# duylebkHCM/doc2tex

Measured on AMD Instinct MI355X. Metric: formulas/s (greedy decode, 128x512 crops), higher is better.
Workload: dtype bf16x3

## Files before the change

doc2tex_amd/_lib.py:

```python
import ctypes as C
import os

_HERE = os.path.dirname(os.path.abspath(__file__))
LIB_PATH = os.path.join(_HERE, "csrc", "libd2t.so")
if os.environ.get("D2T_PROBE_LIB"):
    LIB_PATH = os.path.abspath(os.environ["D2T_PROBE_LIB"])

D2T_OK = 0
D2T_EINVAL, D2T_ENOMEM, D2T_EHIP, D2T_ESTATE = 1, 2, 3, 4
ENC_RESNET, ENC_HYBRID_VIT, ENC_VGG_BILSTM, ENC_RESNET_BILSTM, ENC_VGG = 0, 1, 2, 3, 4
DEC_TFM, DEC_ATTN = 0, 1
ATTN_KEYS_ALL_INIT_MEAN, ATTN_KEYS_NOCLS_INIT_CLS, ATTN_KEYS_ALL_INIT_FIRST = 0, 1, 2
ACT_NONE, ACT_RELU, ACT_GELU = 0, 1, 2
CONV_FP32, CONV_BF16X3, CONV_FP16X2, CONV_MIXED = 0, 1, 2, 3
ATTN_CELL_LOCATION, ATTN_CELL_BAHDANAU = 0, 1
VIT_POS_SINCOS_PREFIX, VIT_POS_LEARNED_INTERP, VIT_POS_LEARNED_PREFIX = 0, 1, 2


class D2TConfig(C.Structure):
    _fields_ = [(n, C.c_int32) for n in (
        "encoder", "in_channels", "backbone_out", "vit_depth", "vit_heads", "vit_dim", "patch_h", "patch_w",
        "max_h", "max_w", "dec_dim", "dec_heads", "dec_layers", "dec_ff", "vocab", "max_seq_len",
        "decoder", "attn_hidden", "attn_kernel_size", "attn_kernel_dim", "attn_keys", "attn_enc_init",
        "attn_coverage", "bilstm_hidden", "batch_max_length", "gcb", "attn_cell", "attn_onehot", "vit_pos",
# ... 95 lines not shown
    "d2t_decode_beam": (_I, [_P, _P, _I, _I, C.POINTER(C.c_int64), C.POINTER(_I), C.POINTER(C.c_float), _P]),
    "d2t_decode_beam_batch": (_I, [_P, _P, _I, _I, _I, C.POINTER(C.c_int64), C.POINTER(_I), C.POINTER(C.c_float), _P]),
    "d2t_decode_beam_batch_ragged": (_I, [_P, _P, _I, C.POINTER(_I), _I, C.POINTER(C.c_int64), C.POINTER(_I), C.POINTER(C.c_float),
                                          _P]),
    "d2t_decode_supports_ragged_beam": (_I, [_P]),
    "d2t_ragged_beam_tables": (_L, [_I, C.POINTER(_I), C.POINTER(_I), C.POINTER(_I)]),
    "d2t_decode_attn_beam_batch": (_I, [_P, _P, _I, _I, _I, C.POINTER(C.c_int64), C.POINTER(_I), C.POINTER(C.c_float), _P]),
    "d2t_decode_attn_beam_batch_alpha": (_I, [_P, _P, _I, _I, _I, C.POINTER(C.c_int64), C.POINTER(_I), C.POINTER(C.c_float), _P,
                                               _P]),
    "d2t_decode_attn_beam_batch_ragged": (_I, [_P, _P, _I, C.POINTER(_I), _I, C.POINTER(C.c_int64), C.POINTER(_I),
                                               C.POINTER(C.c_float), _P, _P]),
    "d2t_decode_attn_supports_ragged_beam": (_I, [_P]),
    "d2t_decode_attn_beam": (_I, [_P, _P, _I, _I, C.POINTER(C.c_int64), C.POINTER(_I), C.POINTER(C.c_float), _P]),
    "d2t_decode_attn_supports_device_beam": (_I, [_P]),
    "d2t_set_attn_beam_device": (_I, [_P, _I]),
    "d2t_decode_attn_beam_device_runs": (_L, [_P]),
    "d2t_decode_attn_beam_batch_submit": (_I, [_P, _P, _I, C.POINTER(_I), _I, _P, _P, _P, _P, _P, C.POINTER(_L)]),
    "d2t_set_conv_precision": (_I, [_P, _I]),
    "d2t_set_mixed_units": (_I, [_P, _I]),
    "d2t_set_reserved_blocks": (_I, [_P, _I]),
    "d2t_set_decode_chains": (_I, [_P, _I]),
    "d2t_set_conv_kernel": (_I, [_P, _I]),
    "d2t_set_conv_fusion": (_I, [_P, _I, _I]),
    "d2t_set_beam_shared_tile": (_I, [_P, _I]),
    "d2t_set_reserved_cus": (_I, [_P, _I]),
    "d2t_train_forward": (_I, [_P, _P, _I, _I, _I, _P, _I, _P, _P]),
    "d2t_train_backward": (_I, [_P, _P, _P]),
    "d2t_train_grad": (_I, [_P, C.c_char_p, _P, C.c_int64, _P]),
    "d2t_reload_weights": (_I, [_P, _I, C.POINTER(C.c_char_p), C.POINTER(C.c_void_p), C.POINTER(C.c_int64), _P]),
    "d2t_train_gather": (_I, [_P, _I, _I, C.POINTER(C.c_char_p), C.POINTER(C.c_int64), C.POINTER(C.c_int64), _P, _P]),
    "d2t_read_weight": (_I, [_P, C.c_char_p, _P, C.c_int64, _P]),
    "d2t_train_set_dropout": (_I, [_P, C.c_float, C.c_uint64]),
    "d2t_train_set_teacher_flags": (_I, [_P, C.c_char_p, _I]),
    "d2t_train_mask_count": (_I, [_P]),
    "d2t_train_decision_count": (_I, [_P]),
    "d2t_train_read_decision": (_I, [_P, _I, _P, C.c_int64, C.POINTER(_I), C.POINTER(C.c_int64), _P]),
    "d2t_train_read_mask": (_I, [_P, _I, _P, C.c_int64, _P]),
    "d2t_train_read_attn_alpha": (_I, [_P, _P, C.c_int64, _P]),
    "d2t_train_release": (None, [_P]),
    "d2t_profile_enable": (_I, [_P, _I]),
    "d2t_profile_read": (_I, [_P, _I, C.POINTER(_I)] + [C.POINTER(_I)] * 3 + [C.POINTER(C.c_float)]),
    "d2t_op_conv2d": (_I, [_P] * 5 + [_I] * 12 + [_P]),
    "d2t_op_conv2d_bf16x3": (_I, [_P] * 5 + [_I] * 12 + [_P]),
    "d2t_op_conv2d_bf16x3_split": (_I, [_P] * 5 + [_I] * 12 + [_P]),
    "d2t_op_conv2d_bf16x3_split_pool": (_I, [_P] * 4 + [_I] * 12 + [_P]),
    "d2t_op_set_conv_kernel": (_I, [_I, _I]),
    "d2t_op_linear": (_I, [_P] * 5 + [_I] * 4 + [_P]),
    "d2t_op_maxpool2x2": (_I, [_P, _P] + [_I] * 8 + [_P]),
    "d2t_op_layernorm": (_I, [_P] * 4 + [_I, _I, C.c_float, _P]),
    "d2t_op_vit_attention": (_I, [_P, _P, _I, _I, _I, _P]),
    "d2t_op_vit_attention_probs": (_I, [_P, _P, _P, _I, _I, _I, _P]),
    "d2t_op_decode_attention": (_I, [_P] * 4 + [_I] * 5 + [_P]),
    "d2t_op_skinny": (_I, [_P] * 6 + [C.c_float, _P, _P] + [_I] * 6 + [_P, _L, _P]),
    "d2t_op_decoder_row": (_I, [_I] + [_P] * 13 + [C.c_float, _P, _P] + [_I] * 7 + [_P, _P, _I, _P, _I, _P]),
    "d2t_op_decoder_row_ragged": (_I, [_I] + [_P] * 13 + [C.c_float, _P, _P] + [_I] * 4 + [C.POINTER(_I), C.POINTER(_I), _P]),
    "d2t_op_decoder_row_ragged_beam": (_I, [_I] + [_P] * 13 + [C.c_float, _P, _P] + [_I] * 5 +
                                       [C.POINTER(_I), C.POINTER(_I), _P, _P, _I, _P]),
    "d2t_op_argmax_embed": (_I, [_P, _I] + [_P] * 13 + [_I] * 6 + [_P]),
    "d2t_op_beam_topk": (_I, [_P, _P, _P] + [_I] * 4 + [_P, _P, _P]),
    "d2t_op_beam_advance": (_I, [_I, _L] + [_P] * 15 + [_I] * 6 + [_P]),
    "d2t_op_beam_ancestry": (_I, [_P, _P, _P, _I, _I, _P, _P, _P, _P, _P]),
    "d2t_op_cache_gather": (_I, [_P, _P, _P] + [_I] * 7 + [_P]),
    "d2t_op_records_split": (_I, [_P, _P, _L, _I, _I, _P]),
    "d2t_op_records_merge": (_I, [_P, _P, _L, _I, _I, _P]),
    "d2t_op_conv_records": (_I, [C.POINTER(D2TOpConvRecordsArgs), _P]),
    "d2t_op_linear_kv": (_I, [_P] * 4 + [_I] * 7 + [_P]),
    "d2t_op_maxpool_records": (_I, [_P, _P] + [_I] * 9 + [_P]),
    "d2t_op_stem_records": (_I, [_P] * 4 + [_I] * 6 + [_P]),
    "d2t_op_pack_conv": (_I, [_P] * 6 + [C.c_float] + [_P] * 6 + [_I] * 4 + [_P]),
    "d2t_ce_forward": (_I, [_P, _P, _P, _P, _I, _I, _L, _P]),
    "d2t_ce_backward": (_I, [_P, _P, _P, _P, _P, _I, _I, _L, _P]),
    "d2t_ce_smooth_forward": (_I, [_P] * 6 + [_I, _I, _L, C.c_float, C.c_float, _I, _L, _P]),
    "d2t_ce_smooth_backward": (_I, [_P] * 7 + [_I, _I, _L, C.c_float, C.c_float, _I, _L, _P]),
    "d2t_optim_create": (_I, [C.POINTER(_P)]),
    "d2t_optim_destroy": (None, [_P]),
    "d2t_optim_last_error": (C.c_char_p, [_P]),
    "d2t_optim_chunk": (_I, []),
    "d2t_optim_step": (_I, [_P, C.POINTER(D2TOptimTensor), _I, _I, C.c_float, _P, _P]),
    "d2t_weight_ptr": (_I, [_P, C.c_char_p, C.POINTER(_P), C.POINTER(_L)]),
    "d2t_metric_edit_distance_workspace": (_I, [_I, _L, C.POINTER(_L)]),
    "d2t_metric_edit_distance": (_I, [_P, _P, _L, _P, _P, _L, _P, _I, _L, _P, _L, _P]),
    "d2t_metric_bleu_counts": (_I, [_P, _I, _P, _I, _I, _L, _I, _P, _P]),
    "d2t_op_train_conv": (_I, [_P] * 14 + [_I] * 13 + [_P]),
    "d2t_op_train_linear": (_I, [_P] * 10 + [_I] * 5 + [_P]),
    "d2t_op_train_layernorm": (_I, [_P] * 8 + [_I, _I, C.c_float, _P]),
    "d2t_op_train_attention": (_I, [_P] * 7 + [_I] * 6 + [_P]),
    "d2t_op_train_maxpool": (_I, [_P] * 4 + [_I] * 8 + [_P]),
    "d2t_op_bilstm": (_I, [_P] * 5 + [_I] * 3 + [_P]),
    "d2t_op_bilstm_hprev": (_I, [_P] * 3 + [_I] * 3 + [_P]),
    "d2t_op_bilstm_bwd": (_I, [_P] * 6 + [_I] * 3 + [_P]),
    "d2t_op_attn_decode": (_I, [C.POINTER(D2TOpAttnDecodeArgs), _P]),
    "d2t_op_attn_decode_ragged": (_I, [C.POINTER(D2TOpAttnDecodeArgs), _P, _P, _I, _P]),
    "d2t_op_attn_decode_group": (_I, [C.POINTER(D2TOpAttnDecodeArgs), _P, _P, _P, _P, _I, _P, _P]),
    "d2t_op_attn_decode_finalize": (_I, [_P, _P] + [_I] * 4 + [_P] * 4),
    "d2t_op_attn_alpha_gather": (_I, [_P] * 4 + [_I] * 4 + [_P]),
    "d2t_op_attn_beam_advance": (_I, [C.POINTER(D2TOpAttnBeamRec), _I, _L, _P]),
    "d2t_op_attn_beam_finish": (_I, [C.POINTER(D2TOpAttnBeamRec)] + [_P] * 6),
    "d2t_op_attn_beam_host_advance": (_I, [C.POINTER(D2TOpAttnBeamRec), _I, _L]),
    "d2t_op_attn_beam_host_finish": (_I, [C.POINTER(D2TOpAttnBeamRec)] + [_P] * 5),
    "d2t_op_attn_lstm_bwd": (_I, [C.POINTER(D2TOpAttnLstmBwdArgs), _P]),
    "d2t_op_loc_unfold_bwd": (_I, [_P, _P, _I, _P, _P, _P, _I, _I, _I] + [_P] * 5),
    "d2t_op_train_gc_pool": (_I, [_P] * 8 + [_I] * 4 + [_P]),
    "d2t_op_train_bcast_add": (_I, [_P] * 6 + [_I] * 3 + [_P]),
    "d2t_op_global_context": (_I, [_P] * 10 + [_I] * 3 + [_P]),
    "d2t_op_embed_train": (_I, [_P] * 4 + [_I] * 4 + [C.c_float, _P]),
    "d2t_op_embed_bwd": (_I, [_P] * 3 + [_I] * 3 + [C.c_float, _I, _P]),
# ... 69 lines not shown
```

doc2tex_amd/csrc/decode.hip:

```cpp
#include <cstdlib>

#include "kernels.h"

namespace d2t {

using f32x4 = __attribute__((ext_vector_type(4))) float;
#ifndef D2T_DECODE_PRIO
#define D2T_DECODE_PRIO 3
#endif

__device__ __forceinline__ void decode_wave_priority() { __builtin_amdgcn_s_setprio(D2T_DECODE_PRIO); }

struct TraceScope {
  unsigned long long* t;
  __device__ __forceinline__ explicit TraceScope(unsigned long long* tr) : t(tr) {
    if (t && threadIdx.x == 0) atomicMin(t, (unsigned long long)__builtin_amdgcn_s_memrealtime());
  }
  __device__ __forceinline__ ~TraceScope() {
    if (t) {
      __syncthreads();
      if (threadIdx.x == 0) atomicMax(t + 1, (unsigned long long)__builtin_amdgcn_s_memrealtime());
    }
  }
};
// ... 82 lines not shown
      s_rstd[tid] = 1.f / sqrtf(t * invK + p.ln_eps);
    }
    __syncthreads();
#pragma unroll
    for (int c = 0; c < NCH; ++c) {
      const float4 g4 = *reinterpret_cast<const float4*>(p.ln_g + k0 + c * 16);
      const float4 b4 = *reinterpret_cast<const float4*>(p.ln_b + k0 + c * 16);
#pragma unroll
      for (int i = 0; i < MT; ++i) {
        const float rs = s_rstd[i * 16 + r];
        a[i][c].x = a[i][c].x * rs * g4.x + b4.x;
        a[i][c].y = a[i][c].y * rs * g4.y + b4.y;
        a[i][c].z = a[i][c].z * rs * g4.z + b4.z;
        a[i][c].w = a[i][c].w * rs * g4.w + b4.w;
      }
    }
  }

  f32x4 acc[MT];
#pragma unroll
  for (int i = 0; i < MT; ++i) acc[i] = f32x4{0.f, 0.f, 0.f, 0.f};
#pragma unroll
  for (int c = 0; c < NCH; ++c) {
#pragma unroll
    for (int i = 0; i < MT; ++i) {
      acc[i] = __builtin_amdgcn_mfma_f32_16x16x4f32(a[i][c].x, b[c].x, acc[i], 0, 0, 0);
      acc[i] = __builtin_amdgcn_mfma_f32_16x16x4f32(a[i][c].y, b[c].y, acc[i], 0, 0, 0);
      acc[i] = __builtin_amdgcn_mfma_f32_16x16x4f32(a[i][c].z, b[c].z, acc[i], 0, 0, 0);
      acc[i] = __builtin_amdgcn_mfma_f32_16x16x4f32(a[i][c].w, b[c].w, acc[i], 0, 0, 0);
    }
  }
#pragma unroll
  for (int i = 0; i < MT; ++i)
#pragma unroll
    for (int reg = 0; reg < 4; ++reg) part[wave][i * 16 + q * 4 + reg][r] = acc[i][reg];
  __syncthreads();

  float* y = p.y;
  if (p.step_ptr) y += (long long)(*p.step_ptr) * p.out_step_stride;
  for (int idx = tid; idx < ROWS * 16; idx += NW * 64) {
    const int row = idx >> 4, col = idx & 15;
    const int m = mbase + row, nn = blockIdx.x * 16 + col;
    if (m >= p.M || nn >= p.N) continue;
    float v = 0.f;
#pragma unroll
    for (int w = 0; w < NW; ++w) v += part[w][row][col];
    v += p.bias ? p.bias[nn] : 0.f;
    if (p.res) v += p.res[(size_t)m * p.ldres + nn];
    y[(size_t)m * p.ldy + nn] = act_fn(v, p.act);
    if (p.ln_out && nn < p.K) {
      const float xv = p.x[(size_t)m * p.ldx + nn];
      p.ln_out[(size_t)m * p.K + nn] = (xv - s_mean[row]) * s_rstd[row] * p.ln_g[nn] + p.ln_b[nn];
    }
  }
}

__global__ __launch_bounds__(256) void skinny_generic_kernel(const SkinnyP p) {
  const int wave = threadIdx.x >> 6, lane = threadIdx.x & 63;
  const int r = lane & 15, q = lane >> 4;
  const int m = blockIdx.y * 64 + wave * 16 + r;
  const int n = blockIdx.x * 16 + r;
  const bool mok = m < p.M, nok = n < p.N;
  const float* xa = p.x + (size_t)(mok ? m : 0) * p.ldx + q * 4;
  const float* wb = p.w + (size_t)(nok ? n : 0) * p.K + q * 4;
  f32x4 acc = {0.f, 0.f, 0.f, 0.f};
  const int KC = p.K >> 4;
  for (int c = 0; c < KC; ++c) {
    float4 a = *reinterpret_cast<const float4*>(xa + c * 16);
    float4 b = *reinterpret_cast<const float4*>(wb + c * 16);
    if (!mok) a = make_float4(0.f, 0.f, 0.f, 0.f);
    if (!nok) b = make_float4(0.f, 0.f, 0.f, 0.f);
    acc = __builtin_amdgcn_mfma_f32_16x16x4f32(a.x, b.x, acc, 0, 0, 0);
    acc = __builtin_amdgcn_mfma_f32_16x16x4f32(a.y, b.y, acc, 0, 0, 0);
    acc = __builtin_amdgcn_mfma_f32_16x16x4f32(a.z, b.z, acc, 0, 0, 0);
    acc = __builtin_amdgcn_mfma_f32_16x16x4f32(a.w, b.w, acc, 0, 0, 0);
  }
  const int nn = blockIdx.x * 16 + r;
  if (nn >= p.N) return;
  float* y = p.y;
  if (p.step_ptr) y += (long long)(*p.step_ptr) * p.out_step_stride;
  const float bias = p.bias ? p.bias[nn] : 0.f;
#pragma unroll
  for (int reg = 0; reg < 4; ++reg) {
    const int mm = blockIdx.y * 64 + wave * 16 + q * 4 + reg;
    if (mm >= p.M) continue;
    float v = acc[reg] + bias;
    if (p.res) v += p.res[(size_t)mm * p.ldres + nn];
    y[(size_t)mm * p.ldy + nn] = act_fn(v, p.act);
  }
}

static int decode_small() {
  static const int v = D2T_PROBE_ENV("D2T_DECODE_SMALL");
  return v;
}

hipError_t launch_skinny(const SkinnyP& p, hipStream_t s) {
  if (p.M <= 0 || p.N <= 0) return hipSuccess;
  if (p.K % 16 != 0 || p.ldx % 4 != 0) return hipErrorInvalidValue;
  if (p.ln_out && (!p.ln_g || p.N < p.K)) return hipErrorInvalidValue;
  const int mt = p.N <= 512 ? 1 : 2;
  const dim3 grid((p.N + 15) / 16, (p.M + 16 * mt - 1) / (16 * mt));
#define D2T_SK(NW, NCH)                                                                                  \
  do {                                                                                                   \
    if (mt == 1) hipLaunchKernelGGL((skinny_splitk_kernel<NW, NCH, 1>), grid, dim3(NW * 64), 0, s, p);   \
    else hipLaunchKernelGGL((skinny_splitk_kernel<NW, NCH, 2>), grid, dim3(NW * 64), 0, s, p);           \
  } while (0)
  if (p.K == 256) D2T_SK(4, 4);
  else if (p.K == 512) D2T_SK(8, 4);
  else if (p.K == 1024 && decode_small() && !p.ln_g && !p.step_ptr) {
    SkinnyP a = p, b = p;
    a.K = 512; a.ldx = p.ldx; a.w = p.w; a.wld = p.K;
    b.K = 512; b.x = p.x + 512; b.w = p.w + 512; b.wld = p.K; b.bias = nullptr; b.res = p.y; b.ldres = p.ldy;
    a.act = ACT_NONE;
    if (p.act != ACT_NONE) return hipErrorInvalidValue;
    hipLaunchKernelGGL((skinny_splitk_kernel<4, 8, 1>), dim3((p.N + 15) / 16, (p.M + 15) / 16), dim3(256), 0, s, a);
    hipLaunchKernelGGL((skinny_splitk_kernel<4, 8, 1>), dim3((p.N + 15) / 16, (p.M + 15) / 16), dim3(256), 0, s, b);
  }
  else if (p.K == 1024) D2T_SK(8, 8);
  else {
    if (p.ln_g) return hipErrorInvalidValue;
    hipLaunchKernelGGL(skinny_generic_kernel, dim3((p.N + 15) / 16, (p.M + 63) / 64), dim3(256), 0, s, p);
  }
#undef D2T_SK
  return hipGetLastError();
}

template <int HD>
__global__ __launch_bounds__(256) void decode_attention_kernel(const DecAttnP p) {
  constexpr int LPK = HD / 4;
  constexpr int KPI = 64 / LPK;
  constexpr int MAXIT = 512 / (KPI * 4);
  __shared__ float w_m[4], w_s[4];
  __shared__ __attribute__((aligned(16))) float w_acc[4][HD];
  const int tid = threadIdx.x, wave = tid >> 6, lane = tid & 63;
  const int kig = lane / LPK, ch = lane % LPK;
  const int b = blockIdx.x / p.heads, head = blockIdx.x % p.heads;
  int L = p.L, t = -1;
  if (p.step_ptr) { t = *p.step_ptr; L = t + 1; }
  float* Kc = p.k + (size_t)b * p.kv_batch_stride + (size_t)head * p.Lmax * HD;
  float* Vc = p.v + (size_t)b * p.kv_batch_stride + (size_t)head * p.Lmax * HD;
  const float* curk = p.cur_k ? p.cur_k + (size_t)b * p.cur_stride + head * HD : nullptr;
  const float* curv = p.cur_v ? p.cur_v + (size_t)b * p.cur_stride + head * HD : nullptr;
  if (curk && t >= 0 && tid < HD) {
    Kc[(size_t)t * HD + tid] = curk[tid];
    Vc[(size_t)t * HD + tid] = curv[tid];
  }
  const float4 q4 = *reinterpret_cast<const float4*>(p.q + (size_t)b * p.q_stride + head * HD + ch * 4);
  const float scale = HD == 32 ? 0.17677669529663687f : 0.125f;
  const int nit = (L + KPI * 4 - 1) / (KPI * 4);

  float sc[MAXIT];
  float mloc = -INFINITY;
// ... 1567 lines not shown
```

doc2tex_amd/csrc/engine_ops.hip:

```cpp
#include <climits>

#include "engine_impl.h"

extern "C" {

int d2t_op_conv2d(const float* x, const float* w, const float* bias, const float* residual, float* y, int32_t B,
                  int32_t H, int32_t W, int32_t Cin, int32_t Cout, int32_t KH, int32_t KW, int32_t SH, int32_t SW,
                  int32_t PH, int32_t PW, int32_t act, d2t_stream stream) {
  if (!x || !w || !y || SH < 1 || SW < 1) return D2T_EINVAL;
  hipStream_t s = (hipStream_t)stream;
  if (Cin == 1 || Cin == 3) {
    if (KH != 3 || KW != 3 || SH != 1 || SW != 1 || PH != 1 || PW != 1 || residual) return D2T_EINVAL;
    return launch_stem(x, w, bias, y, B, Cin, H, W, Cout, act, s) == hipSuccess ? D2T_OK : D2T_EHIP;
  }
  if (Cin % 32) return D2T_EINVAL;
  float* wp = nullptr;
  if (hipMalloc(reinterpret_cast<void**>(&wp), (size_t)Cout * KH * KW * Cin * 4) != hipSuccess) return D2T_ENOMEM;
  ConvP p{};
  p.in = x; p.w = wp; p.bias = bias; p.res = residual; p.out = y;
  conv_shape(p, B, H, W, Cin, Cout, KH, KW, SH, SW, PH, PW);
  p.act = act;
  hipError_t e = launch_repack_ohwi(w, wp, Cout, KH, KW, Cin, s);
  if (e == hipSuccess) e = launch_conv(p, s);
  hipStreamSynchronize(s);
// ... 258 lines not shown
int d2t_op_layernorm(const float* x, const float* gamma, const float* beta, float* y, int32_t rows, int32_t D,
                     float eps, d2t_stream stream) {
  if (!x || !gamma || !beta || !y) return D2T_EINVAL;
  return launch_layernorm(x, gamma, beta, y, rows, D, eps, (hipStream_t)stream) == hipSuccess ? D2T_OK : D2T_EHIP;
}

int d2t_op_global_context(float* x, const float* wg, const float* bg, const float* w1, const float* b1, const float* ln_g,
                          const float* ln_b, const float* w2, const float* b2, float* ctx_out, int32_t B, int32_t HW, int32_t C,
                          d2t_stream stream) {
  if (!x || !wg || !bg || !w1 || !b1 || !ln_g || !ln_b || !w2 || !b2) return D2T_EINVAL;
  if (B < 1 || B > 65535 || HW < 1 || HW > (1 << 24) || C < 4 || C > 512 || C % 4) return D2T_EINVAL;
  hipStream_t s = (hipStream_t)stream;
  const size_t nl = (size_t)B * HW, nc = (size_t)B * C;
  float* buf = nullptr;
  if (hipMalloc(reinterpret_cast<void**>(&buf), (nl + 2 * nc) * 4) != hipSuccess) return D2T_ENOMEM;
  float *logits = buf, *ctx = buf + nl, *y = ctx + nc;
  const GCParams w{wg, bg, w1, b1, ln_g, ln_b, w2, b2};
  hipError_t e = launch_global_context(x, w, logits, ctx, y, B, HW, C, s);
  if (e == hipSuccess && ctx_out) e = hipMemcpyAsync(ctx_out, ctx, nc * 4, hipMemcpyDeviceToDevice, s);
  hipStreamSynchronize(s);
  hipFree(buf);
  return op_status(e);
}

int d2t_op_vit_attention(const float* qkv, float* y, int32_t B, int32_t N, int32_t heads, d2t_stream stream) {
  if (!qkv || !y) return D2T_EINVAL;
  return launch_vit_attention(qkv, y, B, N, heads, (hipStream_t)stream) == hipSuccess ? D2T_OK : D2T_EHIP;
}

int d2t_op_vit_attention_probs(const float* qkv, float* y, float* probs, int32_t B, int32_t N, int32_t heads,
                               d2t_stream stream) {
  if (!qkv || !y || !probs || B < 1 || N < 1 || heads < 1) return D2T_EINVAL;
  return launch_vit_attention_probs(qkv, y, probs, B, N, heads, (hipStream_t)stream) == hipSuccess ? D2T_OK : D2T_EHIP;
}

int d2t_op_decode_attention(const float* q, const float* k, const float* v, float* y, int32_t B, int32_t heads,
                            int32_t hd, int32_t L, int32_t Lmax, d2t_stream stream) {
  if (!q || !k || !v || !y || L > Lmax) return D2T_EINVAL;
  DecAttnP p{};
  p.q = q; p.q_stride = heads * hd; p.k = const_cast<float*>(k); p.v = const_cast<float*>(v);
  p.y = y; p.y_stride = heads * hd; p.B = B; p.heads = heads; p.hd = hd; p.Lmax = Lmax; p.L = L;
  p.kv_batch_stride = (long long)heads * Lmax * hd;
  return launch_decode_attention(p, (hipStream_t)stream) == hipSuccess ? D2T_OK : D2T_EHIP;
}

namespace {
bool fetch_ints(hipStream_t s, const int* dev, size_t n, std::vector<int>* out) {
  out->resize(n);
  if (hipStreamSynchronize(s) != hipSuccess) return false;
  return n == 0 || hipMemcpy(out->data(), dev, n * sizeof(int), hipMemcpyDeviceToHost) == hipSuccess;
}
}

int d2t_op_skinny(const float* x, const float* w, const float* bias, const float* res, const float* ln_g, const float* ln_b,
                  float ln_eps, float* y, float* ln_out, int32_t M, int32_t K, int32_t N, int32_t ldx, int32_t ldy, int32_t act,
                  const int32_t* step, int64_t out_step_stride, d2t_stream stream) {
  if (!x || !w || !y || M < 1 || M > 65535 * 16 || N < 1 || K < 16 || K % 16 || ldx < K || ldx % 4 || ldy < N) return D2T_EINVAL;
  if (act != ACT_NONE && act != ACT_RELU && act != ACT_GELU) return D2T_EINVAL;
  if ((ln_g == nullptr) != (ln_b == nullptr) || (ln_out && !ln_g)) return D2T_EINVAL;
  hipStream_t s = (hipStream_t)stream;
  if (step) {
    std::vector<int> t;
    if (out_step_stride < 0 || !fetch_ints(s, step, 1, &t) || t[0] < 0) return D2T_EINVAL;
  }
  SkinnyP p{};
  p.x = x; p.w = w; p.bias = bias; p.res = res; p.y = y;
  p.M = M; p.K = K; p.N = N; p.ldx = ldx; p.ldy = ldy; p.ldres = N; p.act = act;
  p.step_ptr = step; p.out_step_stride = out_step_stride;
  p.ln_g = ln_g; p.ln_b = ln_b; p.ln_eps = ln_eps; p.ln_out = ln_out;
  const hipError_t e = launch_skinny(p, s);
  return op_status(e);
}

namespace {
struct RowOpTmp { float* buf; float* wv_t; float* ext; };
int row_op_setup(const float* qkv, const float* xres, float* sk, float* sv, const float* ca_in_w, const float* ca_in_b,
                 const float* sa_out_w, const float* sa_out_b, const float* ca_out_w, const float* ca_out_b, const float* ln1_g,
                 const float* ln1_b, float eps, float* y2, const int32_t* step, int M, int D, int Lmax, size_t extra,
                 hipStream_t s, RowOpTmp* t, DecRowP* r, hipError_t* e) {
  const size_t dd = (size_t)D * D;
  t->buf = nullptr;
  if (hipMalloc(reinterpret_cast<void**>(&t->buf), 4 * dd * 4 + extra) != hipSuccess) return D2T_ENOMEM;
  float *wo_t = t->buf, *wq_t = t->buf + dd, *wco_t = t->buf + 2 * dd;
  t->wv_t = t->buf + 3 * dd; t->ext = t->buf + 4 * dd;
  *e = launch_transpose(sa_out_w, wo_t, D, D, s);
  if (*e == hipSuccess) *e = launch_transpose(ca_in_w, wq_t, D, D, s);
  if (*e == hipSuccess) *e = launch_transpose(ca_out_w, wco_t, D, D, s);
  if (*e == hipSuccess) *e = launch_transpose(ca_in_w + 2 * dd, t->wv_t, D, D, s);
  *r = DecRowP{};
  r->qkv = qkv; r->qkv_stride = 3 * D; r->xres = xres;
  r->sk = sk; r->sv = sv; r->s_batch_stride = (long long)Lmax * D; r->s_Lmax = Lmax;
  r->wo_t = wo_t; r->bo = sa_out_b; r->ln1_g = ln1_g; r->ln1_b = ln1_b; r->eps = eps;
  r->wq_t = wq_t; r->bq = ca_in_b; r->wco_t = wco_t; r->bco = ca_out_b;
  r->y2 = y2; r->step_ptr = step; r->M = M; r->D = D; r->heads = 8;
  return D2T_OK;
}
static int row_op_check(hipStream_t s, const int32_t* step, int Lmax, const int32_t* row_map, int M, int samples, const int32_t* anc,
                 int anc_stride, int rows) {
  std::vector<int> h;
  if (!fetch_ints(s, step, 1, &h)) return D2T_EHIP;
  const int t = h[0];
  if (t < 0 || t >= Lmax) return D2T_EINVAL;
  if (row_map) {
    if (!fetch_ints(s, row_map, M, &h)) return D2T_EHIP;
    for (int v : h) if (v < 0 || v >= samples) return D2T_EINVAL;
  }
  if (anc) {
    if (!fetch_ints(s, anc, (size_t)M * anc_stride, &h)) return D2T_EHIP;
    for (int b = 0; b < M; ++b)
      for (int j = 0; j < t; ++j)
        if (h[(size_t)b * anc_stride + j] < 0 || h[(size_t)b * anc_stride + j] >= rows) return D2T_EINVAL;
  }
  return D2T_OK;
}
static bool ragged_slices_ok(const int32_t* row0, const int32_t* len, int n, int mem_rows) {
  for (int i = 0; i < n; ++i)
    if (row0[i] < 0 || len[i] < 1 || len[i] > 4096 || (long long)row0[i] + len[i] > mem_rows) return false;
  return true;
}
static int row_op_finish(hipStream_t s, float* buf, hipError_t e) {
  const hipError_t e2 = hipStreamSynchronize(s);
  hipFree(buf);
  return e == hipErrorInvalidValue ? D2T_EINVAL : (e == hipSuccess && e2 == hipSuccess) ? D2T_OK : D2T_EHIP;
}
// ... 544 lines not shown
```

doc2tex_amd/csrc/kernels.h:

```cpp
#pragma once
#include <hip/hip_runtime.h>
#include <stdint.h>

#pragma GCC visibility push(hidden)
#include "attn_beam_host.h"
#pragma GCC visibility pop

#include <cstdlib>
#ifdef D2T_PROBES
#define D2T_PROBE_ENV(name) (getenv(name) ? atoi(getenv(name)) : 0)
#define D2T_PROBE_ENV_STR(name) getenv(name)
#else
#define D2T_PROBE_ENV(name) 0
#define D2T_PROBE_ENV_STR(name) (static_cast<const char*>(nullptr))
#endif

namespace d2t {

enum { ACT_NONE = 0, ACT_RELU = 1, ACT_GELU = 2 };
enum { STORE_ROWS = 0, STORE_KV = 1 };

struct ConvP {
  const float* in;
  const float* w;
// ... 4 lines not shown
  const uint16_t* res_hi;
  const void* zero16;
  int max_blocks;
  int reserved_cus;
  int wave_prio;
  int pipelined;
  int split_tail;
  int pool2;
  const uint16_t* in2_hi;
  int Cin2;
  int f16;
  int out_fmt, res_fmt;
  const float* bias;
  const float* res;
  const float* row_add;
  float* out;
  int B, H, W, Cin, OH, OW, Cout;
  int KH, KW, SH, SW, PH, PW;
  int M;
  int m_base;
  int K;
  int act;
  int rows_per_img, img_stride, row_off, row_add_off;
  int store_mode, kv_T, kv_heads, kv_hd, kv_B;
};
inline void conv_shape(ConvP& p, int B, int H, int W, int Cin, int Cout, int KH, int KW, int SH, int SW, int PH, int PW,
                       int OH = -1, int OW = -1) {
  p.B = B; p.H = H; p.W = W; p.Cin = Cin; p.Cout = Cout;
  p.KH = KH; p.KW = KW; p.SH = SH; p.SW = SW; p.PH = PH; p.PW = PW;
  p.OH = OH >= 0 ? OH : (H + 2 * PH - KH) / SH + 1;
  p.OW = OW >= 0 ? OW : (W + 2 * PW - KW) / SW + 1;
  p.M = B * p.OH * p.OW; p.K = KH * KW * Cin;
}
inline void linear_shape(ConvP& p, int M, int K, int N) { conv_shape(p, 1, 1, M, K, N, 1, 1, 1, 1, 0, 0); }
hipError_t launch_conv(const ConvP& p, hipStream_t s);
hipError_t launch_conv_bf16x3(const ConvP& p, hipStream_t s);
hipError_t launch_conv_bf16x3p(const ConvP& p, hipStream_t s);
hipError_t launch_split_bf16(const float* w, uint16_t* hi, uint16_t* lo, size_t n, hipStream_t s);
hipError_t launch_split_f16(const float* w, uint16_t* hi, uint16_t* lo, size_t n, hipStream_t s);

struct SkinnyP {
  const float* x; const float* w; const float* bias; const float* res; float* y;
  int M, K, N;
  int ldx, ldy, ldres;
  int wld;
  unsigned long long* trace;
  const int* stop_at; const int* cur_step;
  int act;
  const int* step_ptr;
  long long out_step_stride;
  const float* ln_g; const float* ln_b; float ln_eps; float* ln_out;
};
hipError_t launch_skinny(const SkinnyP& p, hipStream_t s);

hipError_t launch_stem(const float* img, const float* w, const float* bias, float* out, int B, int Cin, int H, int W, int Cout,
                       int act, hipStream_t s);
hipError_t launch_stem_split(const float* img, const float* w, const float* bias, uint16_t* out, int B, int Cin, int H, int W,
                             int Cout, int act, hipStream_t s, int fmt = 0);
hipError_t launch_split_act(const float* x, uint16_t* planes, size_t rows, int C, hipStream_t s, int fmt = 0);
hipError_t launch_merge_act(const uint16_t* planes, float* x, size_t rows, int C, hipStream_t s, int fmt = 0);
hipError_t launch_maxpool(const float* x, float* y, int B, int H, int W, int C, int SH, int SW, int PH, int PW,
                          hipStream_t s);
hipError_t launch_maxpool_split(const uint16_t* x, uint16_t* y, int B, int H, int W, int C, int SH, int SW, int PH,
                                int PW, hipStream_t s, int fmt = 0);
hipError_t launch_maxpool_k(const float* x, float* y, int B, int H, int W, int C, int KH, int KW, int SH, int SW,
                            int PH, int PW, hipStream_t s);
hipError_t launch_mean_h(const float* x, float* y, int B, int H, int W, int C, hipStream_t s);

hipError_t launch_bilstm(const float* g, const float* whh_t, float* out, int B, int T, int H, hipStream_t s);

struct AttnDecP {
  const float* mem; int T; int D;
  int key_off;
  int init_mode;
  const float* kp;
  const float* wq_t; const float* bq;
  const float* wloc; const float* bloc; int taps;
  const float* wscore; float bscore;
  const float* wx_t; const float* bx;
  const float* wg_t; const float* bg;
  const float* wih_t; const float* bih; const float* wic_t; const float* bic;
  const float* emb;
  const float* tokgate;
  float* probs; int64_t* tokens; int* end_step;
  int B, S, V, H, E, coverage, end_token;
  int step_mode, first;
  const float *st_h_in, *st_c_in, *st_mem_in;
  float *st_h_out, *st_c_out, *st_mem_out;
  const int64_t* tok_in;
  const int* row_sample;
  const int64_t* teacher;
  const uint8_t* use_teacher;
  const uint8_t* out_dropmask;
  float out_dropscale;
  int64_t* sv_tok;
  float *sv_hprev, *sv_cprev, *sv_hafter, *sv_cafter;
  float* sv_gates;
  float* sv_alpha;
  float* sv_hq;
  float* sv_x;
  unsigned long long* exit_state;
  const int* smp_row0;
  const int* smp_T;
  int st_ld;
  const int* guard;
  const int* grp_row0;
// ... 276 lines not shown
```

include/d2t.h:

```cpp
#ifndef D2T_H
#define D2T_H

#include <stdint.h>

#ifdef __cplusplus
extern "C" {
#endif

typedef struct d2t_ctx d2t_ctx;
typedef void* d2t_stream;

enum {
  D2T_OK = 0,
  D2T_EINVAL = 1,
  D2T_ENOMEM = 2,
  D2T_EHIP = 3,
  D2T_ESTATE = 4
};

enum {
  D2T_ENC_RESNET = 0,
  D2T_ENC_HYBRID_VIT = 1,
  D2T_ENC_VGG_BILSTM = 2,
  D2T_ENC_RESNET_BILSTM = 3,
// ... 136 lines not shown
int d2t_set_reserved_cus(d2t_ctx* ctx, int32_t cus);
int d2t_set_decode_chains(d2t_ctx* ctx, int32_t chains);

int d2t_train_forward(d2t_ctx* ctx, const float* image, int32_t B, int32_t H, int32_t W, const int64_t* tgt, int32_t L,
                      float* logits, d2t_stream stream);
int d2t_train_backward(d2t_ctx* ctx, const float* dlogits, d2t_stream stream);
int d2t_train_grad(d2t_ctx* ctx, const char* name, float* dst, int64_t numel, d2t_stream stream);
int d2t_train_gather(d2t_ctx* ctx, int32_t source, int32_t n, const char* const* names, const int64_t* offsets,
                     const int64_t* numels, float* flat, d2t_stream stream);
int d2t_reload_weights(d2t_ctx* ctx, int32_t n, const char* const* names, const float* const* srcs, const int64_t* numels,
                       d2t_stream stream);
int d2t_read_weight(d2t_ctx* ctx, const char* name, float* dst, int64_t numel, d2t_stream stream);
int d2t_train_set_dropout(d2t_ctx* ctx, float p, uint64_t seed);
int d2t_train_set_teacher_flags(d2t_ctx* ctx, const uint8_t* flags, int32_t n);
int d2t_train_mask_count(d2t_ctx* ctx);
int d2t_train_decision_count(d2t_ctx* ctx);
int d2t_train_read_decision(d2t_ctx* ctx, int32_t index, uint8_t* dst, int64_t numel, int32_t* is_pool_out,
                            int64_t* numel_out, d2t_stream stream);
int d2t_train_read_mask(d2t_ctx* ctx, int32_t index, uint8_t* dst, int64_t numel, d2t_stream stream);
int d2t_train_read_attn_alpha(d2t_ctx* ctx, float* dst, int64_t numel, d2t_stream stream);
void d2t_train_release(d2t_ctx* ctx);

int d2t_profile_enable(d2t_ctx* ctx, int32_t on);
int d2t_profile_read(d2t_ctx* ctx, int32_t max_records, int32_t* n, int32_t* M, int32_t* N, int32_t* K, float* ms);

int d2t_op_conv2d(const float* x, const float* w, const float* bias, const float* residual, float* y, int32_t B,
                  int32_t H, int32_t W, int32_t Cin, int32_t Cout, int32_t KH, int32_t KW, int32_t SH, int32_t SW,
                  int32_t PH, int32_t PW, int32_t act, d2t_stream stream);
int d2t_op_conv2d_bf16x3(const float* x, const float* w, const float* bias, const float* residual, float* y, int32_t B,
                         int32_t H, int32_t W, int32_t Cin, int32_t Cout, int32_t KH, int32_t KW, int32_t SH,
                         int32_t SW, int32_t PH, int32_t PW, int32_t act, d2t_stream stream);
int d2t_op_set_conv_kernel(int32_t kind, int32_t reserved_cus);
int d2t_op_conv2d_bf16x3_split_pool(const float* x, const float* w, const float* bias, float* y, int32_t B, int32_t H, int32_t W,
                                    int32_t Cin, int32_t Cout, int32_t KH, int32_t KW, int32_t SH, int32_t SW, int32_t PH,
                                    int32_t PW, int32_t act, d2t_stream stream);
int d2t_op_conv2d_bf16x3_split(const float* x, const float* w, const float* bias, const float* residual, float* y,
                               int32_t B, int32_t H, int32_t W, int32_t Cin, int32_t Cout, int32_t KH, int32_t KW,
                               int32_t SH, int32_t SW, int32_t PH, int32_t PW, int32_t act, d2t_stream stream);
int d2t_op_linear(const float* x, const float* w, const float* bias, const float* residual, float* y, int32_t M,
                  int32_t K, int32_t N, int32_t act, d2t_stream stream);
int d2t_op_maxpool2x2(const float* x, float* y, int32_t B, int32_t H, int32_t W, int32_t C, int32_t SH, int32_t SW,
                      int32_t PH, int32_t PW, d2t_stream stream);
int d2t_op_layernorm(const float* x, const float* gamma, const float* beta, float* y, int32_t rows, int32_t D,
                     float eps, d2t_stream stream);
int d2t_op_vit_attention(const float* qkv, float* y, int32_t B, int32_t N, int32_t heads, d2t_stream stream);
int d2t_op_vit_attention_probs(const float* qkv, float* y, float* probs, int32_t B, int32_t N, int32_t heads,
                               d2t_stream stream);
int d2t_op_decode_attention(const float* q, const float* k, const float* v, float* y, int32_t B, int32_t heads,
                            int32_t hd, int32_t L, int32_t Lmax, d2t_stream stream);

int d2t_op_skinny(const float* x, const float* w, const float* bias, const float* res, const float* ln_g, const float* ln_b,
                  float ln_eps, float* y, float* ln_out, int32_t M, int32_t K, int32_t N, int32_t ldx, int32_t ldy, int32_t act,
                  const int32_t* step, int64_t out_step_stride, d2t_stream stream);
int d2t_op_decoder_row(int32_t kind, const float* qkv, const float* xres, float* sk, float* sv, const float* mem,
                       const float* ca_in_w, const float* ca_in_b, const float* sa_out_w, const float* sa_out_b,
                       const float* ca_out_w, const float* ca_out_b, const float* ln1_g, const float* ln1_b, float eps, float* y2,
                       const int32_t* step, int32_t M, int32_t D, int32_t T, int32_t Lmax, int32_t rows, int32_t samples,
                       int32_t one_row, const int32_t* row_map, const int32_t* anc, int32_t anc_stride, const int32_t* seg,
                       int32_t nsamples, d2t_stream stream);
int d2t_op_decoder_row_ragged(int32_t kind, const float* qkv, const float* xres, float* sk, float* sv, const float* mem,
                              const float* ca_in_w, const float* ca_in_b, const float* sa_out_w, const float* sa_out_b,
                              const float* ca_out_w, const float* ca_out_b, const float* ln1_g, const float* ln1_b, float eps,
                              float* y2, const int32_t* step, int32_t M, int32_t Lmax, int32_t rows, int32_t mem_rows,
                              const int32_t* row0, const int32_t* len, d2t_stream stream);
int d2t_op_decoder_row_ragged_beam(int32_t kind, const float* qkv, const float* xres, float* sk, float* sv, const float* mem,
                                   const float* ca_in_w, const float* ca_in_b, const float* sa_out_w, const float* sa_out_b,
                                   const float* ca_out_w, const float* ca_out_b, const float* ln1_g, const float* ln1_b, float eps,
                                   float* y2, const int32_t* step, int32_t M, int32_t Lmax, int32_t rows, int32_t mem_rows,
                                   int32_t samples, const int32_t* row0, const int32_t* len, const int32_t* row_map,
                                   const int32_t* anc, int32_t anc_stride, d2t_stream stream);
int d2t_op_argmax_embed(const float* logits, int32_t S, int64_t* tokens, int32_t* ended, int32_t* end_count, int32_t* steps_done,
                        int32_t* step, int32_t* done_count, int32_t* batch_end_count, int32_t* batch_steps_done,
                        int32_t* batches_done, int32_t* stop_at, const float* emb, const float* pe, float* x, int32_t B, int32_t V,
                        int32_t d, int32_t end_token, int32_t rows_per_batch, int32_t n_batches, d2t_stream stream);
int d2t_op_beam_topk(const float* logits, const float* scores, const int32_t* seg, int32_t N, int32_t rows, int32_t V, int32_t kmax,
                     float* topv, int32_t* topi, d2t_stream stream);
int d2t_op_beam_advance(int32_t init, int64_t go_token, int32_t* ctrl, int64_t* tok, float* scores, int32_t* map, int32_t* prev,
                        int32_t* seg, int32_t* comp_n, int32_t* fin, int32_t* comp_t, int32_t* comp_par, float* comp_score,
                        int32_t* hist_par, int32_t* hist_tok, const float* topv, const int32_t* topi, int32_t N, int32_t beam,
                        int32_t cap, int32_t V, int32_t S, int32_t end_token, d2t_stream stream);
int d2t_op_beam_ancestry(const int32_t* anc_old, int32_t* anc_new, const int32_t* prev, int32_t rows, int32_t stride,
                         const int32_t* step_in, int32_t* step_out, const int32_t* rows_ptr, const int32_t* stop,
                         d2t_stream stream);
int d2t_op_cache_gather(const float* src, float* dst, const int32_t* prev, int32_t slabs, int32_t cap, int32_t M, int32_t heads,
                        int32_t Lmax, int32_t hd, int32_t rows, d2t_stream stream);

int d2t_op_records_split(const float* x, uint16_t* planes, int64_t rows, int32_t C, int32_t fmt, d2t_stream stream);
int d2t_op_records_merge(const uint16_t* planes, float* x, int64_t rows, int32_t C, int32_t fmt, d2t_stream stream);
typedef struct d2t_op_conv_records_args {
  const uint16_t* x_rec; const float* x_f32; const uint16_t* x2_rec;
  const float* w; const float* w2; const float* bias; const float* bias2;
  const uint16_t* res_rec; const float* res_f32; const float* row_add;
  uint16_t* out_rec; float* out_f32;
  int32_t in_fmt, res_fmt, out_fmt;
  int32_t B, H, W, Cin, Cin2, Cout, KH, KW, SH, SW, PH, PW, OH, OW, act, pool2;
  int32_t rows_per_img, img_stride, row_off, row_add_off, row_add_rows, out_rows;
  int32_t kind, split_tail;
} d2t_op_conv_records_args;
int d2t_op_conv_records(const d2t_op_conv_records_args* a, d2t_stream stream);
int d2t_op_linear_kv(const float* x, const float* w, const float* bias, float* y, int32_t K, int32_t N, int32_t kv_B, int32_t kv_T,
                     int32_t heads, int32_t hd, int32_t bf16x3, d2t_stream stream);
int d2t_op_maxpool_records(const uint16_t* x, uint16_t* y, int32_t B, int32_t H, int32_t W, int32_t C, int32_t SH, int32_t SW,
                           int32_t PH, int32_t PW, int32_t fmt, d2t_stream stream);
int d2t_op_stem_records(const float* img, const float* w, const float* bias, uint16_t* out, int32_t B, int32_t Cin, int32_t H,
                        int32_t W, int32_t act, int32_t fmt, d2t_stream stream);
int d2t_op_pack_conv(const float* w_oihw, const float* conv_bias, const float* bn_w, const float* bn_b, const float* bn_mean,
// ... 150 lines not shown
```

Before: 1622.

## Add register-tiled wide skinny GEMM kernel for large-M decode projections

Adds a skinny_wide_kernel that tiles each block over multiple 16-row and 16-column MFMA tiles and keeps the activation and weight chunks in registers. Each loaded row is reused across several output columns, with optional fused layernorm and split-K reduction through shared memory. Auto-selection uses it for K of 256 or 1024 when M is at least 384, and a new form-selecting entry point is exposed for testing. This is meant to cut redundant activation loads and launch count in batched decode, at the cost of high register and shared-memory use and reduced occupancy.

```diff
diff --git a/doc2tex_amd/_lib.py b/doc2tex_amd/_lib.py
--- a/doc2tex_amd/_lib.py
+++ b/doc2tex_amd/_lib.py
@@ -171,6 +171,7 @@
     "d2t_op_vit_attention_probs": (_I, [_P, _P, _P, _I, _I, _I, _P]),
     "d2t_op_decode_attention": (_I, [_P] * 4 + [_I] * 5 + [_P]),
     "d2t_op_skinny": (_I, [_P] * 6 + [C.c_float, _P, _P] + [_I] * 6 + [_P, _L, _P]),
+    "d2t_op_skinny_form": (_I, [_P] * 6 + [C.c_float, _P, _P] + [_I] * 6 + [_P, _L, _I, _P]),
     "d2t_op_decoder_row": (_I, [_I] + [_P] * 13 + [C.c_float, _P, _P] + [_I] * 7 + [_P, _P, _I, _P, _I, _P]),
     "d2t_op_decoder_row_ragged": (_I, [_I] + [_P] * 13 + [C.c_float, _P, _P] + [_I] * 4 + [C.POINTER(_I), C.POINTER(_I), _P]),
     "d2t_op_decoder_row_ragged_beam": (_I, [_I] + [_P] * 13 + [C.c_float, _P, _P] + [_I] * 5 +
diff --git a/doc2tex_amd/csrc/decode.hip b/doc2tex_amd/csrc/decode.hip
--- a/doc2tex_amd/csrc/decode.hip
+++ b/doc2tex_amd/csrc/decode.hip
@@ -158,6 +158,170 @@
       const float xv = p.x[(size_t)m * p.ldx + nn];
       p.ln_out[(size_t)m * p.K + nn] = (xv - s_mean[row]) * s_rstd[row] * p.ln_g[nn] + p.ln_b[nn];
     }
+  }
+}
+
+template <int NW, int NCH, int TM, int TN, int NWV>
+__global__ __launch_bounds__(NWV * 64) void skinny_wide_kernel(const SkinnyP p) {
+  if (p.stop_at && *p.stop_at && *p.cur_step >= *p.stop_at) return;
+  decode_wave_priority();
+  TraceScope trace_(p.trace);
+  constexpr int KS = NCH * 16, ROWS = 16 * TM, COLS = 16 * TN;
+  constexpr int G = NWV / NW;
+  constexpr int TMW = TM / G;
+  constexpr int WG = NWV / 4;
+  constexpr int NE = TM * TN / WG;
+  static_assert(NW * G == NWV && TMW * G == TM && NE * WG == TM * TN && WG * 4 == NWV, "the waves share the units evenly");
+  __shared__ float part[NW][TM * TN][4][64];
+  __shared__ float stat[NW][ROWS];
+  __shared__ float s_mean[ROWS], s_rstd[ROWS];
+  const int tid = threadIdx.x, wave = tid >> 6, lane = tid & 63;
+  const int r = lane & 15, q = lane >> 4;
+  const int w = wave % NW, i0 = (wave / NW) * TMW;
+  const int mbase = blockIdx.y * ROWS, nbase = blockIdx.x * COLS;
+  const int k0 = w * KS + q * 4;
+
+  const long long yoff = p.step_ptr ? (long long)(*p.step_ptr) * p.out_step_stride : 0;
+  float bias_v[NE], res_v[NE];
+#pragma unroll
+  for (int e = 0; e < NE; ++e) {
+    const int st = (wave >> 2) + WG * e;
+    const int m = mbase + (st / TN) * 16 + q * 4 + (wave & 3), nn = nbase + (st % TN) * 16 + r;
+    const bool ok = m < p.M && nn < p.N;
+    bias_v[e] = p.bias && ok ? p.bias[nn] : 0.f;
+    res_v[e] = p.res && ok ? p.res[(size_t)m * p.ldres + nn] : 0.f;
+  }
+  float4 g4[NCH], b4[NCH];
+  if (p.ln_g) {
+#pragma unroll
+    for (int c = 0; c < NCH; ++c) {
+      g4[c] = *reinterpret_cast<const float4*>(p.ln_g + k0 + c * 16);
+      b4[c] = *reinterpret_cast<const float4*>(p.ln_b + k0 + c * 16);
+    }
+  }
+  float4 a[TMW][NCH], b[TN][NCH];
+#pragma unroll
+  for (int i = 0; i < TMW; ++i) {
+    const int m = mbase + (i0 + i) * 16 + r;
+    const bool mok = m < p.M;
+    const float* src = p.x + (size_t)(mok ? m : 0) * p.ldx + k0;
+#pragma unroll
+    for (int c = 0; c < NCH; ++c) {
+      a[i][c] = *reinterpret_cast<const float4*>(src + c * 16);
+      if (!mok) a[i][c] = make_float4(0.f, 0.f, 0.f, 0.f);
+    }
+  }
+#pragma unroll
+  for (int c = 0; c < NCH; ++c) {
+#pragma unroll
+    for (int j = 0; j < TN; ++j) {
+      const int n = nbase + j * 16 + r;
+      const bool nok = n < p.N;
+      b[j][c] = *reinterpret_cast<const float4*>(p.w + (size_t)(nok ? n : 0) * (p.wld ? p.wld : p.K) + k0 + c * 16);
+      if (!nok) b[j][c] = make_float4(0.f, 0.f, 0.f, 0.f);
+    }
+  }
+
+  if (p.ln_g) {
+    const float invK = 1.f / (float)p.K;
+#pragma unroll
+    for (int i = 0; i < TMW; ++i) {
+      float s = 0.f;
+#pragma unroll
+      for (int c = 0; c < NCH; ++c) s += (a[i][c].x + a[i][c].y) + (a[i][c].z + a[i][c].w);
+      s += __shfl_xor(s, 16, 64);
+      s += __shfl_xor(s, 32, 64);
+      if (q == 0) stat[w][(i0 + i) * 16 + r] = s;
+    }
+    __syncthreads();
+    if (tid < ROWS) {
+      float t = 0.f;
+#pragma unroll
+      for (int ww = 0; ww < NW; ++ww) t += stat[ww][tid];
+      s_mean[tid] = t * invK;
+    }
+    __syncthreads();
+#pragma unroll
+    for (int i = 0; i < TMW; ++i) {
+      const float mu = s_mean[(i0 + i) * 16 + r];
+      float s = 0.f;
+#pragma unroll
+      for (int c = 0; c < NCH; ++c) {
+        a[i][c].x -= mu; a[i][c].y -= mu; a[i][c].z -= mu; a[i][c].w -= mu;
+        s += (a[i][c].x * a[i][c].x + a[i][c].y * a[i][c].y) + (a[i][c].z * a[i][c].z + a[i][c].w * a[i][c].w);
+      }
+      s += __shfl_xor(s, 16, 64);
+      s += __shfl_xor(s, 32, 64);
+      if (q == 0) stat[w][(i0 + i) * 16 + r] = s;
+    }
+    __syncthreads();
+    if (tid < ROWS) {
+      float t = 0.f;
+#pragma unroll
+      for (int ww = 0; ww < NW; ++ww) t += stat[ww][tid];
+      s_rstd[tid] = 1.f / sqrtf(t * invK + p.ln_eps);
+    }
+    __syncthreads();
+#pragma unroll
+    for (int i = 0; i < TMW; ++i) {
+      const float rs = s_rstd[(i0 + i) * 16 + r];
+#pragma unroll
+      for (int c = 0; c < NCH; ++c) {
+        a[i][c].x = a[i][c].x * rs * g4[c].x + b4[c].x;
+        a[i][c].y = a[i][c].y * rs * g4[c].y + b4[c].y;
+        a[i][c].z = a[i][c].z * rs * g4[c].z + b4[c].z;
+        a[i][c].w = a[i][c].w * rs * g4[c].w + b4[c].w;
+      }
+    }
+    if (p.ln_out) {
+#pragma unroll
+      for (int i = 0; i < TMW; ++i) {
+        const int m = mbase + (i0 + i) * 16 + r;
+#pragma unroll
+        for (int c = 0; c < NCH; ++c) {
+          const int k = k0 + c * 16;
+          if (m < p.M && k / COLS == (int)blockIdx.x) *reinterpret_cast<float4*>(p.ln_out + (size_t)m * p.K + k) = a[i][c];
+        }
+      }
+    }
+  }
+
+  f32x4 acc[TMW][TN];
+#pragma unroll
+  for (int i = 0; i < TMW; ++i)
+#pragma unroll
+    for (int j = 0; j < TN; ++j) acc[i][j] = f32x4{0.f, 0.f, 0.f, 0.f};
+#define D2T_WIDE_MFMA(f)                                                                                     \
+  _Pragma("unroll") for (int i = 0; i < TMW; ++i) _Pragma("unroll") for (int j = 0; j < TN; ++j)             \
+    acc[i][j] = __builtin_amdgcn_mfma_f32_16x16x4f32(a[i][c].f, b[j][c].f, acc[i][j], 0, 0, 0)
+#pragma unroll
+  for (int c = 0; c < NCH; ++c) {
+    D2T_WIDE_MFMA(x);
+    D2T_WIDE_MFMA(y);
+    D2T_WIDE_MFMA(z);
+    D2T_WIDE_MFMA(w);
+  }
+#undef D2T_WIDE_MFMA
+#pragma unroll
+  for (int i = 0; i < TMW; ++i)
+#pragma unroll
+    for (int j = 0; j < TN; ++j)
+#pragma unroll
+      for (int reg = 0; reg < 4; ++reg) part[w][(i0 + i) * TN + j][reg][lane] = acc[i][j][reg];
+  __syncthreads();
+
+  float* y = p.y + yoff;
+#pragma unroll
+  for (int e = 0; e < NE; ++e) {
+    const int st = (wave >> 2) + WG * e;
+    const int m = mbase + (st / TN) * 16 + q * 4 + (wave & 3), nn = nbase + (st % TN) * 16 + r;
+    if (m >= p.M || nn >= p.N) continue;
+    float v = 0.f;
+#pragma unroll
+    for (int ww = 0; ww < NW; ++ww) v += part[ww][st][wave & 3][lane];
+    v += bias_v[e];
+    if (p.res) v += res_v[e];
+    y[(size_t)m * p.ldy + nn] = act_fn(v, p.act);
   }
 }
 
@@ -201,10 +365,30 @@
   return v;
 }
 
-hipError_t launch_skinny(const SkinnyP& p, hipStream_t s) {
+template <int NW, int NCH, int TM, int TN, int NWV>
+static void launch_skinny_wide(const SkinnyP& p, hipStream_t s) {
+  const dim3 grid((p.N + 16 * TN - 1) / (16 * TN), (p.M + 16 * TM - 1) / (16 * TM));
+  hipLaunchKernelGGL((skinny_wide_kernel<NW, NCH, TM, TN, NWV>), grid, dim3(NWV * 64), 0, s, p);
+}
+
+hipError_t launch_skinny(const SkinnyP& p, hipStream_t s) { return launch_skinny_form(p, SKINNY_FORM_AUTO, s); }
+
+hipError_t launch_skinny_form(const SkinnyP& p, int form, hipStream_t s) {
   if (p.M <= 0 || p.N <= 0) return hipSuccess;
   if (p.K % 16 != 0 || p.ldx % 4 != 0) return hipErrorInvalidValue;
   if (p.ln_out && (!p.ln_g || p.N < p.K)) return hipErrorInvalidValue;
+  const bool wide_k = p.K == 256 || p.K == 512 || p.K == 1024;
+  if (form == SKINNY_FORM_AUTO)
+    form = (p.K == 256 || p.K == 1024) && p.M >= SKINNY_WIDE_MIN_M && !decode_small() ? SKINNY_FORM_WIDE : SKINNY_FORM_SPLITK;
+  if (form == SKINNY_FORM_WIDE) {
+    if (!wide_k) return hipErrorInvalidValue;
+    if (p.K == 256 && p.N > 512) launch_skinny_wide<4, 4, 2, 4, 4>(p, s);
+    else if (p.K == 256) launch_skinny_wide<4, 4, 2, 2, 4>(p, s);
+    else if (p.K == 512) launch_skinny_wide<8, 4, 2, 2, 8>(p, s);
+    else launch_skinny_wide<8, 8, 2, 1, 8>(p, s);
+    return hipGetLastError();
+  }
+  if (form != SKINNY_FORM_SPLITK) return hipErrorInvalidValue;
   const int mt = p.N <= 512 ? 1 : 2;
   const dim3 grid((p.N + 15) / 16, (p.M + 16 * mt - 1) / (16 * mt));
 #define D2T_SK(NW, NCH)                                                                                  \
diff --git a/doc2tex_amd/csrc/engine_ops.hip b/doc2tex_amd/csrc/engine_ops.hip
--- a/doc2tex_amd/csrc/engine_ops.hip
+++ b/doc2tex_amd/csrc/engine_ops.hip
@@ -334,9 +334,10 @@
 }
 }
 
-int d2t_op_skinny(const float* x, const float* w, const float* bias, const float* res, const float* ln_g, const float* ln_b,
-                  float ln_eps, float* y, float* ln_out, int32_t M, int32_t K, int32_t N, int32_t ldx, int32_t ldy, int32_t act,
-                  const int32_t* step, int64_t out_step_stride, d2t_stream stream) {
+namespace {
+int op_skinny(const float* x, const float* w, const float* bias, const float* res, const float* ln_g, const float* ln_b,
+              float ln_eps, float* y, float* ln_out, int32_t M, int32_t K, int32_t N, int32_t ldx, int32_t ldy, int32_t act,
+              const int32_t* step, int64_t out_step_stride, int form, d2t_stream stream) {
   if (!x || !w || !y || M < 1 || M > 65535 * 16 || N < 1 || K < 16 || K % 16 || ldx < K || ldx % 4 || ldy < N) return D2T_EINVAL;
   if (act != ACT_NONE && act != ACT_RELU && act != ACT_GELU) return D2T_EINVAL;
   if ((ln_g == nullptr) != (ln_b == nullptr) || (ln_out && !ln_g)) return D2T_EINVAL;
@@ -350,8 +351,24 @@
   p.M = M; p.K = K; p.N = N; p.ldx = ldx; p.ldy = ldy; p.ldres = N; p.act = act;
   p.step_ptr = step; p.out_step_stride = out_step_stride;
   p.ln_g = ln_g; p.ln_b = ln_b; p.ln_eps = ln_eps; p.ln_out = ln_out;
-  const hipError_t e = launch_skinny(p, s);
+  const hipError_t e = launch_skinny_form(p, form, s);
   return op_status(e);
+}
+}
+
+int d2t_op_skinny(const float* x, const float* w, const float* bias, const float* res, const float* ln_g, const float* ln_b,
+                  float ln_eps, float* y, float* ln_out, int32_t M, int32_t K, int32_t N, int32_t ldx, int32_t ldy, int32_t act,
+                  const int32_t* step, int64_t out_step_stride, d2t_stream stream) {
+  return op_skinny(x, w, bias, res, ln_g, ln_b, ln_eps, y, ln_out, M, K, N, ldx, ldy, act, step, out_step_stride, SKINNY_FORM_AUTO,
+                   stream);
+}
+
+int d2t_op_skinny_form(const float* x, const float* w, const float* bias, const float* res, const float* ln_g,
+                       const float* ln_b, float ln_eps, float* y, float* ln_out, int32_t M, int32_t K, int32_t N, int32_t ldx,
+                       int32_t ldy, int32_t act, const int32_t* step, int64_t out_step_stride, int32_t form,
+                       d2t_stream stream) {
+  if (form != SKINNY_FORM_SPLITK && form != SKINNY_FORM_WIDE) return D2T_EINVAL;
+  return op_skinny(x, w, bias, res, ln_g, ln_b, ln_eps, y, ln_out, M, K, N, ldx, ldy, act, step, out_step_stride, form, stream);
 }
 
 namespace {
diff --git a/doc2tex_amd/csrc/kernels.h b/doc2tex_amd/csrc/kernels.h
--- a/doc2tex_amd/csrc/kernels.h
+++ b/doc2tex_amd/csrc/kernels.h
@@ -80,6 +80,9 @@
   const float* ln_g; const float* ln_b; float ln_eps; float* ln_out;
 };
 hipError_t launch_skinny(const SkinnyP& p, hipStream_t s);
+enum { SKINNY_FORM_AUTO = -1, SKINNY_FORM_SPLITK = 0, SKINNY_FORM_WIDE = 1 };
+constexpr int SKINNY_WIDE_MIN_M = 384;
+hipError_t launch_skinny_form(const SkinnyP& p, int form, hipStream_t s);
 
 hipError_t launch_stem(const float* img, const float* w, const float* bias, float* out, int B, int Cin, int H, int W, int Cout,
                        int act, hipStream_t s);
diff --git a/include/d2t.h b/include/d2t.h
--- a/include/d2t.h
+++ b/include/d2t.h
@@ -212,6 +212,10 @@
 int d2t_op_skinny(const float* x, const float* w, const float* bias, const float* res, const float* ln_g, const float* ln_b,
                   float ln_eps, float* y, float* ln_out, int32_t M, int32_t K, int32_t N, int32_t ldx, int32_t ldy, int32_t act,
                   const int32_t* step, int64_t out_step_stride, d2t_stream stream);
+int d2t_op_skinny_form(const float* x, const float* w, const float* bias, const float* res, const float* ln_g,
+                       const float* ln_b, float ln_eps, float* y, float* ln_out, int32_t M, int32_t K, int32_t N, int32_t ldx,
+                       int32_t ldy, int32_t act, const int32_t* step, int64_t out_step_stride, int32_t form,
+                       d2t_stream stream);
 int d2t_op_decoder_row(int32_t kind, const float* qkv, const float* xres, float* sk, float* sv, const float* mem,
                        const float* ca_in_w, const float* ca_in_b, const float* sa_out_w, const float* sa_out_b,
                        const float* ca_out_w, const float* ca_out_b, const float* ln1_g, const float* ln1_b, float eps, float* y2,
```

After: 1645 (median of 6 runs). +1.4%, better.
